# LulinZhang/BRDF-NeRF

Hardware: AMD Instinct MI355X
Metric: train rays/sec (+ MFMA% of roofline), spsbrdf-nerf 64 samples/ray, 1/2/4/8 MI355X (higher is better)
Workload: dtype bf16; 1 GPU; BASELINE config 2: Djibouti-shaped synthetic rays, spsbrdf-nerf lambert train step (pass1 64 + guided 64 samples/ray, F=512, 8 Siren layers, PE10, ds_lambda=10), 4096 rays/GPU/step (4096 rays per global step, weak scaling); rays_per_gpu=4096, n_samples=64, guided_samples=64, parallelism=dp1, settle_steps=224

## Files before the change

### brdf_nerf_amd/csrc/field.h

```cpp
#pragma once
#include "common.h"

#define BN_MAX_PASS 3
#define BN_DPH (3 * BN_MAX_HEADS)
#define BN_SINGLE_HEAD_NTW(NT) ((NT) > 1 ? (NT) / 2 : 1)

struct FieldGeom {
  int F, L, skip, pe_freqs, act;
  int P;
  int KP;
  int NT;
  int BM, waves;
  int dsz;
  int H2;
  int n_heads, n_pass;
  int pass_heads[BN_MAX_PASS];
  int pass_N[BN_MAX_PASS];
  int pass_NTW[BN_MAX_PASS];
  int head_col[BN_MAX_HEADS];
  int C;
  int ch_normal_an, ch_normal_lr;
  int fold;
  int DD, KD, dir_freqs, TD, KT0;
};
// ... 90 lines not shown
  for (int l = 0; l < g.L; ++l) pl->bwd_trunk[l] = l >= 1 ? take(g.F, g.F) : 0;
  pl->bwd_feats = g.fold ? 0 : take(g.F, g.F);
  for (int p = 0; p < g.n_pass; ++p) pl->bwd_head[p] = take(g.F, g.pass_N[p]);
  pl->bwd_pe[0] = take(g.KP, g.F);
  pl->bwd_pe[1] = g.skip > 0 ? take(g.KP, g.F) : 0;
  pl->total = off;
}

struct StashLayout {
  size_t gscale;
  size_t sraw;
  size_t nraw;
  size_t dpre_trunk;
  size_t dpre_head;
  size_t pe;
  size_t dirpe;
  size_t Y[BN_MAX_LAYERS];
  size_t D[BN_MAX_LAYERS];
  size_t feats;
  size_t G[BN_MAX_PASS];
  size_t DG[BN_MAX_PASS];
  size_t dZ[BN_MAX_LAYERS];
  size_t dfeats;
  size_t dG[BN_MAX_PASS];
  size_t gradx;
  size_t sbar;
  size_t sprime;
  size_t gbar_pe;
  size_t adj_delta[BN_MAX_LAYERS];
  size_t adj_a[BN_MAX_LAYERS];
  size_t adj_abar[BN_MAX_LAYERS + 1];
  size_t adj_zbar[BN_MAX_LAYERS];
  size_t wgpart, wgpart_bytes;
  size_t total;
  int64_t Mpad;
};

static inline int64_t bn_wgrad_splits(bool half, int64_t tiles, int64_t Mpad, int64_t *m_per_block) {
  const int64_t stage = half ? 64 : 32;
  const int64_t min_mpb = half ? 512 : 256;
  int64_t n_split = (half ? (Mpad <= 327680 ? BN_W2_BLOCKS : 2 * BN_W2_BLOCKS) : 2048) / (tiles > 0 ? tiles : 1);
  if (n_split < 1) n_split = 1;
  int64_t mpb = ceil_div64(ceil_div64(Mpad, n_split), stage) * stage;
  if (mpb < min_mpb) mpb = min_mpb;
  if (m_per_block) *m_per_block = mpb;
  return ceil_div64(Mpad, mpb);
}
static inline size_t bn_wgpart_bytes(const FieldGeom &g, int64_t Mpad, size_t esz) {
  const bool half = esz != 4;
  const int64_t tl = half ? 256 : 128, ft = (g.F + tl - 1) / tl;
  const int64_t tiles_bound = (2 * g.L + 12) * ft * ft;
  const int64_t grid_bound = half ? 2 * BN_W2_BLOCKS : 2048;
  int64_t slabs = tiles_bound > grid_bound ? tiles_bound : grid_bound;
  const int64_t by_points = tiles_bound * bn_wgrad_splits(half, 1, Mpad, nullptr);
  if (by_points < slabs) slabs = by_points;
  const size_t wg = (size_t)slabs * (size_t)(tl * tl + tl) * 4;
  int64_t sk_splits = ceil_div64(Mpad, g.BM);
  if (sk_splits > 256) sk_splits = 256;
  const size_t sk = (size_t)10 * (size_t)sk_splits * (4 * 512 + 4) * 4;
  return wg > sk ? wg : sk;
}

static inline void bn_make_stash_layout(const FieldGeom &g, int64_t n_points, int BM, size_t esz, StashLayout *s) {
  const size_t dsz = (size_t)g.dsz;
  int64_t Mpad = ceil_div64(n_points, BM) * BM;
  s->Mpad = Mpad;
  size_t off = 0;
  auto take = [&](size_t bytes) { size_t o = off; off += bn_pad(bytes, 256); return o; };
  s->gscale = take(256);
  s->sraw = take((size_t)Mpad * 4);
  s->nraw = take((size_t)Mpad * 16);
  s->dpre_trunk = take((size_t)Mpad * 16);
  s->dpre_head = take((size_t)Mpad * BN_DPH * 4);
  s->pe = take((size_t)Mpad * g.KP * esz);
  s->dirpe = g.KD > 0 ? take((size_t)Mpad * g.KD * esz) : 0;
  for (int l = 0; l < g.L; ++l) s->Y[l] = take((size_t)Mpad * g.F * esz);
  for (int l = 0; l < g.L; ++l) s->D[l] = take((size_t)Mpad * g.F * dsz);
  s->feats = take((size_t)Mpad * g.F * esz);
  for (int p = 0; p < BN_MAX_PASS; ++p) {
    s->G[p] = s->DG[p] = s->dG[p] = 0;
    if (p < g.n_pass) {
      s->G[p] = take((size_t)Mpad * g.F * esz);
      s->DG[p] = take((size_t)Mpad * g.F * dsz);
    }
  }
  for (int l = 0; l < g.L; ++l) s->dZ[l] = take((size_t)Mpad * g.F * esz);
  s->dfeats = take((size_t)Mpad * g.F * esz);
  for (int p = 0; p < g.n_pass; ++p) s->dG[p] = take((size_t)Mpad * g.pass_N[p] * esz);
  s->gradx = s->sbar = s->sprime = s->gbar_pe = 0;
  for (int l = 0; l < BN_MAX_LAYERS; ++l) s->adj_delta[l] = s->adj_a[l] = s->adj_abar[l] = s->adj_zbar[l] = 0;
  s->adj_abar[BN_MAX_LAYERS] = 0;
  if (g.ch_normal_an >= 0) {
    s->gradx = take((size_t)Mpad * 16);
    s->sbar = take((size_t)Mpad * 4);
    s->sprime = take((size_t)Mpad * 4);
    s->gbar_pe = take((size_t)Mpad * g.KP * esz);
    for (int l = 0; l < g.L; ++l) {
      s->adj_delta[l] = take((size_t)Mpad * g.F * esz);
      s->adj_a[l] = take((size_t)Mpad * g.F * esz);
      s->adj_abar[l + 1] = take((size_t)Mpad * g.F * esz);
      s->adj_zbar[l] = take((size_t)Mpad * g.F * esz);
    }
  }
  s->wgpart_bytes = bn_wgpart_bytes(g, Mpad, esz);
  s->wgpart = take(s->wgpart_bytes);
  s->total = off;
}

static inline void bn_stash_layout_at(const FieldGeom &g, const bn_points *pts, int BM, size_t esz, StashLayout *s) {
  const int64_t total = pts->total_points > 0 ? pts->total_points : pts->n_points;
  bn_make_stash_layout(g, total, BM, esz, s);
  const size_t off = (size_t)pts->point_offset;
  if (off == 0) return;
  const size_t dsz = (size_t)g.dsz, F = (size_t)g.F;
  s->sraw += off * 4; s->nraw += off * 16; s->dpre_trunk += off * 16; s->dpre_head += off * BN_DPH * 4;
  s->pe += off * g.KP * esz;
  if (g.KD > 0) s->dirpe += off * g.KD * esz;
  for (int l = 0; l < g.L; ++l) { s->Y[l] += off * F * esz; s->D[l] += off * F * dsz; s->dZ[l] += off * F * esz; }
  s->feats += off * F * esz; s->dfeats += off * F * esz;
  for (int p = 0; p < g.n_pass; ++p) { s->G[p] += off * F * esz; s->DG[p] += off * F * dsz; s->dG[p] += off * g.pass_N[p] * esz; }
  if (g.ch_normal_an >= 0) {
    s->gradx += off * 16; s->sbar += off * 4; s->sprime += off * 4; s->gbar_pe += off * g.KP * esz;
    for (int l = 0; l < g.L; ++l) {
      s->adj_delta[l] += off * F * esz; s->adj_a[l] += off * F * esz; s->adj_abar[l + 1] += off * F * esz; s->adj_zbar[l] += off * F * esz;
    }
  }
  s->Mpad = ceil_div64(pts->n_points, BM) * BM;
}
```

### brdf_nerf_amd/csrc/field_bwd.hip

```cpp
#include "field_kernels.h"
#include "field_wgrad.h"

int bn_field_adjoint_backward(const bn_field_desc *desc, const bn_field_params *params, const void *packed, const bn_points *pts,
                              const float *d_out, void *stash, void *stream);

__device__ unsigned int g_bwd_fault;
unsigned int bn_bwd_fault_read(hipStream_t) {
  unsigned int v = 0u;
  if (hipMemcpyFromSymbol(&v, HIP_SYMBOL(g_bwd_fault), sizeof(unsigned int), 0, hipMemcpyDeviceToHost) != hipSuccess) return 0x80000000u;
  return v;
}
const unsigned int *bn_bwd_fault_ptr() {
  void *p = nullptr;
  return hipGetSymbolAddress(&p, HIP_SYMBOL(g_bwd_fault)) == hipSuccess ? (const unsigned int *)p : nullptr;
}

BN_PH_DEFINE_READER(bn_debug_phase_read_bwd)
BN_CLK_DEFINE(bn_debug_clock_read_bwd)

struct BwdArgs {
  FieldGeom g;
  bn_field_desc d;
  bn_field_params p;
  PackedLayout pl;
// ... 190 lines not shown
  const float gs = chain_scale(A.amax);
  if (tid < 16) WR[tid] = 0;
  if (tid < BM) {
    const int m = tid;
    const int64_t gm = m0 + m;
    float dph[BN_DPH], dpt[4];
    bwd_dpre(A, gm, dph, dpt);
    float *sh = (float *)(A.stash + A.sl.dpre_head) + gm * BN_DPH;
    float *st = (float *)(A.stash + A.sl.dpre_trunk) + gm * 4;
#pragma unroll
    for (int i = 0; i < BN_DPH; ++i) { DPH[m * BN_DPH + i] = dph[i] * gs; sh[i] = dph[i]; }
#pragma unroll
    for (int i = 0; i < 4; ++i) { DPT[m * 4 + i] = dpt[i] * gs; st[i] = dpt[i]; }
  }
  __syncthreads();
  BN_PH(0)

  const int ncol0 = wave * 32 * NT;
  const bool wave_on = ncol0 < F;
  const int n_on = F / (32 * NT) < WAVES ? F / (32 * NT) : WAVES;
  const bool ride = NT == 2 ? true : tile_copy_exact(F, n_on, WAVES);
  f32x16 acc[NT][MT];
  zero_acc<MT, NT>(acc);
  const float zr = (A.an && A.amax) ? gs / grad_scale_from(A.amax + 1, BN_GS_TARGET_ADJ) : 1.f;

  for (int p = 0; p < g.n_pass; ++p) {
    if (g.pass_heads[p] == 2) bwd_head_dG<T, MT, NT, D16>(A, p, ACT, DPH, m0, tile);
    else bwd_head_dG<T, MT, BN_SINGLE_HEAD_NTW(NT), D16>(A, p, ACT, DPH, m0, tile);
    BN_PH(1)
    __syncthreads();
    BN_PH(2)
    BN_PH(3)
    const int KSp = g.pass_N[p] / 16;
    tile_to_global<T>(ACT, LDA, (T *)(A.stash + A.sl.dG[p]) + (size_t)m0 * g.pass_N[p], g.pass_N[p], BM, g.pass_N[p]);
    if (wave_on) gemm_seg<T, MT, NT, DP>(acc, packed + A.pl.bwd_head[p] + (size_t)(ncol0 / 32) * KSp * 512, KSp, ACT, LDA, lane);
    BN_PH(4)
    __syncthreads();
    BN_PH(5)
  }
  if (wave_on && !g.fold) {
#pragma unroll
    for (int nt = 0; nt < NT; ++nt)
#pragma unroll
      for (int gq = 0; gq < 4; ++gq) {
        const int n = ncol0 + nt * 32 + 8 * gq + 4 * h;
#pragma unroll
        for (int mt = 0; mt < MT; ++mt) {
          const int m = mt * 32 + r;
          *(vec4 *)(ACT + (size_t)m * LDA + n) =
              to_vec4(T(), acc[nt][mt][4 * gq], acc[nt][mt][4 * gq + 1], acc[nt][mt][4 * gq + 2], acc[nt][mt][4 * gq + 3]);
        }
      }
  }
  BN_PH(6)
  __syncthreads();
  BN_PH(7)
  BN_PH(8)

  constexpr bool NATZ = Elem<T>::kNativeY;
#ifndef BN_BWD_NO_PINGPONG
  constexpr bool PING = NT == 2 && WAVES == 8 && Elem<T>::kFastMath;
#else
  constexpr bool PING = false;
#endif
  const int grp = wave >> 2;
  const int wave_u = __builtin_amdgcn_readfirstlane(wave);
  DPiece<DK> dpre[NT][MT];
  auto load_D = [&](int lo, int nt0, int nt1) {
    const char *Ds = A.stash + A.sl.D[lo] + (size_t)tile * dtile_bytes<DK>(BM, F);
#pragma unroll
    for (int nt = 0; nt < NT; ++nt)
#pragma unroll
      for (int mt = 0; mt < MT; ++mt) {
        if (nt < nt0 || nt >= nt1) continue;
#ifdef BN_PROBE_NO_D
        if constexpr (std::is_same<DK, DK8>::value) { dpre[nt][mt].w = u32x4{0x80808080u + (unsigned)lane, 0x90909090u, 0xa0a0a0a0u, 0xb0b0b0b0u}; continue; }
#endif
        dpre[nt][mt] = dpiece_load<DK>(Ds + dpiece_off<DK, MT, NT>(wave, nt, mt, lane));
      }
  };
  auto epilogue = [&](int lo, auto top_tag) {
    constexpr bool top = decltype(top_tag)::value;
    const bool nlr = g.ch_normal_lr >= 0;
    const float dscale = (g.act == BN_ACT_SIN && lo == 0) ? 30.f : 1.f;
    const auto Zr = stash_rsrc(A.stash + A.sl.dZ[lo] + (size_t)tile * BM * F * sizeof(T));
    const int voff = lane * 16;
    typedef typename Elem<T>::wide WT;
    constexpr bool ZPRE = sizeof(WT) == 2;
    u32x4 zraw[ZPRE ? NT : 1][ZPRE ? MT : 1][2];
    if constexpr (ZPRE) {
      if (A.an) {
        const WT *Zb = (const WT *)(A.stash + A.sl.adj_zbar[lo]) + (size_t)tile * BM * F;
#pragma unroll
        for (int nt = 0; nt < NT; ++nt)
#pragma unroll
          for (int mt = 0; mt < MT; ++mt)
#pragma unroll
            for (int gp = 0; gp < 2; ++gp) zraw[nt][mt][gp] = stash_load((const u32x4 *)(Zb + native_off8<MT, NT>(wave, nt, mt, gp, lane)));
      }
    }
#pragma unroll
    for (int nt = 0; nt < NT; ++nt)
#pragma unroll
      for (int mt = 0; mt < MT; ++mt) {
        const int m = mt * 32 + r;
#pragma unroll
        for (int gp = 0; gp < 2; ++gp) {
          const int n0 = ncol0 + nt * 32 + 16 * gp + 4 * h;
          float dv[8], v[8];
          dpiece_get<DK>(dpre[nt][mt], gp, g.act, dscale, dv);
#pragma unroll
          for (int e = 0; e < 8; ++e) v[e] = acc[nt][mt][8 * gp + e];
          if constexpr (top) {
            const float ds = DPT[m * 4], a0 = DPT[m * 4 + 1], a1 = DPT[m * 4 + 2], a2 = DPT[m * 4 + 3];
#pragma unroll
            for (int half = 0; half < 2; ++half) {
              const int n = n0 + 8 * half;
              const f32x4 ws = *(const f32x4 *)(A.p.sigma_w + n);
#pragma unroll
              for (int e = 0; e < 4; ++e) v[4 * half + e] += ws[e] * ds;
              if (nlr) {
                const f32x4 wn0 = *(const f32x4 *)(A.p.normal_w + n), wn1 = *(const f32x4 *)(A.p.normal_w + F + n),
                            wn2 = *(const f32x4 *)(A.p.normal_w + 2 * F + n);
#pragma unroll
                for (int e = 0; e < 4; ++e) v[4 * half + e] += wn0[e] * a0 + wn1[e] * a1 + wn2[e] * a2;
              }
            }
          }
#pragma unroll
          for (int e = 0; e < 8; ++e) v[e] *= dv[e];
          if (A.an) {
            float zb[8];
            if constexpr (ZPRE) {
              const auto zq = __builtin_bit_cast(bf16x8, zraw[nt][mt][gp]);
#pragma unroll
              for (int e = 0; e < 8; ++e) zb[e] = (float)zq[e];
            } else {
              ld8((const WT *)(A.stash + A.sl.adj_zbar[lo]) + (size_t)tile * BM * F + native_off8<MT, NT>(wave, nt, mt, gp, lane), zb);
            }
#pragma unroll
            for (int e = 0; e < 8; ++e) v[e] += zb[e] * zr;
          }
          if constexpr (NATZ) {
            const typename Elem<T>::frag q = cvt8(T(), v);
            *(vec4 *)(ACT + (size_t)m * LDA + n0) = __builtin_shufflevector(q, q, 0, 1, 2, 3);
            *(vec4 *)(ACT + (size_t)m * LDA + n0 + 8) = __builtin_shufflevector(q, q, 4, 5, 6, 7);
            stash_store_buf(Zr, voff, ((((wave_u * NT + nt) * MT + mt) * 2 + gp) * 1024), q);
          } else {
            *(vec4 *)(ACT + (size_t)m * LDA + n0) = to_vec4(T(), v[0], v[1], v[2], v[3]);
            *(vec4 *)(ACT + (size_t)m * LDA + n0 + 8) = to_vec4(T(), v[4], v[5], v[6], v[7]);
          }
        }
      }
  };
  {
    if (!g.fold) {
      zero_acc<MT, NT>(acc);
      T *fdst = (T *)(A.stash + A.sl.dfeats) + (size_t)m0 * F;
      if (!ride) tile_to_global<T>(ACT, LDA, fdst, F, BM, F);
      if (wave_on) {
        load_D(g.L - 1, 0, NPRE);
        const size_t off = A.pl.bwd_feats + (size_t)(ncol0 / 32) * KSF * 512;
        if (ride) {
          TileCopyExact<T> zcopy(ACT, LDA, fdst, F, F, tid, WAVES * 64);
          gemm_seg<T, MT, NT, DP>(acc, packed + off, KSF, ACT, LDA, lane, zcopy);
        } else {
          gemm_seg<T, MT, NT, DP>(acc, packed + off, KSF, ACT, LDA, lane);
        }
        load_D(g.L - 1, NPRE, NT);
      }
    } else if (wave_on) {
      load_D(g.L - 1, 0, NT);
    }
    BN_PH(9)
    __syncthreads();
    BN_PH(10)
    if (wave_on) epilogue(g.L - 1, std::true_type());
    BN_PH(11)
    __syncthreads();
    BN_PH(12)
  }
  for (int l = g.L - 1; l >= 1; --l) {
    const int it = g.L - 1 - l;
    const int lo = l - 1;
    zero_acc<MT, NT>(acc);
    T *zdst = (T *)(A.stash + A.sl.dZ[l]) + (size_t)m0 * F;
// ... 100 lines not shown
  bn_make_stash_layout(g, pts->n_points, BM, esz, &a.sl);
  const int64_t tiles = ceil_div64(pts->n_points, BM);
  hipStream_t st = (hipStream_t)stream;
  int rc;
  float *amax = f16m ? (float *)((char *)stash + a.sl.gscale) : nullptr;
  a.amax = amax;
  const unsigned amax_grid = (unsigned)(ceil_div64(pts->n_points, 256) < 1024 ? ceil_div64(pts->n_points, 256) : 1024);
  if (parts & BN_BWD_CHAIN) {
  if (f16m) {
    clear_words_kernel<<<1, 64, 0, st>>>((unsigned int *)amax, 4);
    BN_LAUNCH_CHECK("clear amax");
    if (a.an) {
      grad_amax_kernel<1><<<amax_grid, 256, 0, st>>>(a, amax);
      BN_LAUNCH_CHECK("grad_amax<1>");
    }
  }
  if (a.an) {
    rc = bn_field_adjoint_backward(desc, params, packed, pts, d_out, stash, stream);
    if (rc) return rc;
  }
  if (f16m) {
    grad_amax_kernel<0><<<amax_grid, 256, 0, st>>>(a, amax);
    BN_LAUNCH_CHECK("grad_amax<0>");
  }
  rc = [&]() -> int { BN_DISPATCH_TILE(desc->dtype, g, launch_bwd, (a, tiles, st)); }();
  if (rc) return rc;
  }

  const StashLayout &sl = a.sl;
  char *S = (char *)stash;
  const int F = g.F, P0 = g.P;
  WgradArgs w;
  w.n_jobs = 0; w.Mpad = sl.Mpad; w.tile0[0] = 0; w.amax = amax; w.part = nullptr; w.n_split = 1;
  int scale_sel = 1;
  int b_native = 0;
  int a_native = 0;
  int part = BN_BWD_WGRAD_TRUNK;
  auto add = [&](const void *A_, int lda, int a0, const void *B_, int ldb, int b0, float *C, int ldc, float *bias, int N, int K) {
    if (!C || !(parts & part)) return;
    WgradJob &j = w.job[w.n_jobs];
    j.scale_sel = scale_sel;
    j.b_native = (b_native ? WG_B_NATIVE : 0) | (a_native ? WG_A_NATIVE : 0); j.b_bm = BM; j.b_F = F; j.b_bm_shift = BM == 128 ? 7 : 6;
    j.A = A_; j.B = B_; j.C = C; j.bias = bias; j.lda = lda; j.ldb = ldb; j.ldc = ldc; j.a_col0 = a0; j.b_col0 = b0; j.N = N; j.K = K;
    w.tile0[w.n_jobs + 1] = w.tile0[w.n_jobs] + ((N + 127) / 128) * ((K + 127) / 128);
    ++w.n_jobs;
  };
  const int naty = bf ? 1 : 0;
  a_native = naty;
  for (int l = 0; l < g.L; ++l) {
    const void *dZ = S + sl.dZ[l];
    b_native = 0;
    if (l == 0) add(dZ, F, 0, S + sl.pe, g.KP, 0, G->trunk_w[l], P0, G->trunk_b[l], F, P0);
    else if (l == g.skip) {
      add(dZ, F, 0, S + sl.pe, g.KP, 0, G->trunk_w[l], F + P0, G->trunk_b[l], F, P0);
      b_native = naty;
      add(dZ, F, 0, S + sl.Y[l - 1], F, 0, G->trunk_w[l] ? G->trunk_w[l] + P0 : nullptr, F + P0, nullptr, F, F);
    } else {
      b_native = naty;
      add(dZ, F, 0, S + sl.Y[l - 1], F, 0, G->trunk_w[l], F, G->trunk_b[l], F, F);
    }
  }
  a_native = 0;
  b_native = naty;
  part = BN_BWD_WGRAD_HEADS;
  if (!g.fold) add(S + sl.dfeats, F, 0, S + sl.Y[g.L - 1], F, 0, G->feats_w, F, G->feats_b, F, F);
  part = BN_BWD_WGRAD_TRUNK;
  b_native = 0;
  if (a.an) {
    scale_sel = 2;
    for (int l = 0; l < g.L; ++l) {
      const void *dl = S + sl.adj_delta[l];
      if (l == 0) add(dl, F, 0, S + sl.gbar_pe, g.KP, 0, G->trunk_w[l], P0, nullptr, F, P0);
      else if (l == g.skip) {
        add(dl, F, 0, S + sl.gbar_pe, g.KP, 0, G->trunk_w[l], F + P0, nullptr, F, P0);
        add(dl, F, 0, S + sl.adj_abar[l], F, 0, G->trunk_w[l] ? G->trunk_w[l] + P0 : nullptr, F + P0, nullptr, F, F);
      } else add(dl, F, 0, S + sl.adj_abar[l], F, 0, G->trunk_w[l], F, nullptr, F, F);
    }
  }
  scale_sel = 1;
  part = BN_BWD_WGRAD_HEADS;
  for (int hd = 0; hd < g.n_heads; ++hd) {
    const int p = hd / 2, hl = hd % 2;
    b_native = g.fold ? naty : 0;
    add(S + sl.dG[p], g.pass_N[p], hl * g.H2, S + (g.fold ? sl.Y[g.L - 1] : sl.feats), F, 0, G->head_w1[hd], F, G->head_b1[hd], g.H2, F);
  }
  if (g.DD > 0 && G->head0_wdir) {
    b_native = 0; scale_sel = 1;
    add(S + sl.dG[0], g.pass_N[0], 0, S + sl.dirpe, g.KD, 0, G->head0_wdir, (int)G->head0_wdir_ld, nullptr, g.H2, g.DD);
  }
  if (g.TD > 0 && G->head1_wt) {
    b_native = 0; scale_sel = 1;
    add(S + sl.dG[0], g.pass_N[0], g.H2, S + sl.dirpe, g.KD, g.KT0, G->head1_wt, (int)G->head1_wt_ld, nullptr, g.H2, g.TD);
  }
  BN_REQUIRE(w.n_jobs <= BN_MAX_WGRAD_JOBS, "field_backward: too many wgrad jobs");
  float *wgpart = (float *)(S + sl.wgpart);
  if (w.n_jobs > 0)
    if (int e = bn_launch_wgrad(w, bf, f16m, sl.Mpad, wgpart, sl.wgpart_bytes, st)) return e;
  if (!(parts & BN_BWD_SKINNY)) return 0;
  SkinnyArgs s;
  s.n_jobs = 0; s.Mpad = sl.Mpad; s.amax = amax; s.part = nullptr;
  for (int i = 0; i < BN_MAX_SKINNY_JOBS; ++i) { s.job[i].scale_sel = 0; s.job[i].unit_dpre = 0; }
  {
    SkinnyJob &j = s.job[s.n_jobs];
    j.X = S + sl.Y[g.L - 1]; j.ldx = F; j.x_col0 = 0; j.K = F; j.dpre = (const float *)(S + sl.dpre_trunk); j.ldp = 4; j.p_col0 = 0;
    j.nc = g.ch_normal_lr >= 0 ? 4 : 1; j.native = 0;
    if (naty) { j.native = 1; j.bm = BM; j.ntw = g.NT; j.tstride = BM * F; }
    for (int c = 0; c < 4; ++c) { j.out[c] = nullptr; j.bias[c] = nullptr; }
    j.out[0] = G->sigma_w; j.bias[0] = G->sigma_b;
    if (g.ch_normal_lr >= 0) {
      BN_REQUIRE(G->normal_w && G->normal_b, "field_backward: normal grads missing");
      for (int c = 0; c < 3; ++c) { j.out[1 + c] = G->normal_w + (size_t)c * F; j.bias[1 + c] = G->normal_b + c; }
    }
    if (j.out[0]) ++s.n_jobs;
  }
  if (a.an && G->sigma_w) {
    SkinnyJob &j = s.job[s.n_jobs++];
// ... 40 lines not shown
```

### brdf_nerf_amd/csrc/field_kernels.h

```cpp
#pragma once
#include "field.h"
#include "instrument.h"

typedef __attribute__((ext_vector_type(4))) unsigned int u32x4;
typedef __attribute__((ext_vector_type(2))) unsigned int u32x2;
template <typename V> __device__ __forceinline__ void stash_store(V *p, const V &v) {
#ifdef BN_NO_NT_STASH
  *p = v;
#else
  __builtin_nontemporal_store(v, p);
#endif
}
template <typename V> __device__ __forceinline__ V stash_load(const V *p) {
#ifdef BN_NO_NT_STASH
  return *p;
#else
  return __builtin_nontemporal_load(p);
#endif
}

__device__ __forceinline__ auto stash_rsrc(const void *base) {
  const unsigned long long b = (unsigned long long)base;
  const unsigned int lo = __builtin_amdgcn_readfirstlane((unsigned int)b), hi = __builtin_amdgcn_readfirstlane((unsigned int)(b >> 32));
  return __builtin_amdgcn_make_buffer_rsrc((void *)(((unsigned long long)hi << 32) | lo), 0, 0x7fffffff, 0x00020000);
// ... 246 lines not shown
    if constexpr (std::is_same<std::decay_t<Side>, NoSide>::value) {
      if (KS == 16) { gemm_fixed<T, MT, NTW, D, 16, 0>(acc, wp, KS, 0, bsrc, ldb, lane, NoMid()); return; }
    }
  }
  gemm_seg<T, MT, NTW, DP>(acc, wp, KS, bsrc, ldb, lane, side);
}

template <int MT, int NTW> __device__ __forceinline__ void zero_acc(f32x16 (&acc)[NTW][MT]) {
#pragma unroll
  for (int nt = 0; nt < NTW; ++nt)
#pragma unroll
    for (int mt = 0; mt < MT; ++mt)
#pragma unroll
      for (int i = 0; i < 16; ++i) acc[nt][mt][i] = 0.f;
}

template <int MT, int NTW> __device__ __forceinline__ size_t native_off8(int wave, int nt, int mt, int gp, int lane) {
  return ((((size_t)(wave * NTW + nt) * MT + mt) * 2 + gp) * 64 + lane) * 8;
}
__device__ __forceinline__ bf16x8 cvt8(bf16, const float (&v)[8]) {
  bf16x8 o;
#pragma unroll
  for (int i = 0; i < 8; ++i) o[i] = (bf16)v[i];
  return o;
}
__device__ __forceinline__ f16x8 cvt8(f16, const float (&v)[8]) {
  const f32x8 f = {v[0], v[1], v[2], v[3], v[4], v[5], v[6], v[7]};
  return __builtin_convertvector(f, f16x8);
}
__device__ __forceinline__ f32x8 cvt8(float, const float (&v)[8]) {
  const f32x8 f = {v[0], v[1], v[2], v[3], v[4], v[5], v[6], v[7]};
  return f;
}
__device__ __forceinline__ void st_frag(bf16 *p, const bf16x8 &o) { stash_store((bf16x8 *)p, o); }
__device__ __forceinline__ void st_frag(f16 *p, const f16x8 &o) { stash_store((f16x8 *)p, o); }
__device__ __forceinline__ void st_frag(float *p, const f32x8 &o) {
  stash_store((f32x4 *)p, f32x4{o[0], o[1], o[2], o[3]});
  stash_store((f32x4 *)(p + 4), f32x4{o[4], o[5], o[6], o[7]});
}
template <typename T> __device__ __forceinline__ void st8(T *p, const float (&v)[8]) { st_frag(p, cvt8(T(), v)); }
__device__ __forceinline__ void ld8(const bf16 *p, float (&v)[8]) {
  const bf16x8 o = stash_load((const bf16x8 *)p);
#pragma unroll
  for (int i = 0; i < 8; ++i) v[i] = (float)o[i];
}
__device__ __forceinline__ void ld8(const f16 *p, float (&v)[8]) {
  const f16x8 o = stash_load((const f16x8 *)p);
#pragma unroll
  for (int i = 0; i < 8; ++i) v[i] = (float)o[i];
}
__device__ __forceinline__ void ld8(const float *p, float (&v)[8]) {
  const f32x4 a = stash_load((const f32x4 *)p), b = stash_load((const f32x4 *)(p + 4));
#pragma unroll
  for (int i = 0; i < 4; ++i) { v[i] = a[i]; v[4 + i] = b[i]; }
}

template <typename DK> struct DPiece { u32x4 w; };
template <> struct DPiece<DK16> { u32x4 w[2]; };
template <> struct DPiece<DK32> { f32x4 v[4]; };
template <typename DK> __host__ __device__ constexpr size_t dk_bytes() { return std::is_same<DK, DK32>::value ? 4 : (std::is_same<DK, DK16>::value ? 2 : 1); }
template <typename DK> __host__ __device__ constexpr size_t dtile_bytes(int BM, int F) { return (size_t)BM * F * dk_bytes<DK>(); }
template <typename DK, int MT, int NTW> __device__ __forceinline__ size_t dpiece_off(int wave, int nt, int mt, int lane) {
  return ((size_t)(wave * NTW + nt) * MT + mt) * (1024 * dk_bytes<DK>()) + (size_t)lane * (std::is_same<DK, DK32>::value ? 64 : 16);
}
__device__ __forceinline__ unsigned int d8_pack4(float c0, float c1, float c2, float c3) {
  const unsigned int lo = __builtin_bit_cast(unsigned int, __builtin_amdgcn_cvt_pknorm_i16(c0, c1)),
// ... 102 lines not shown
```

### brdf_nerf_amd/csrc/field_wgrad.h

```cpp
#pragma once
#include <hip/hip_runtime.h>
#include <stdint.h>

struct WgradJob {
  const void *A;
  const void *B;
  float *C;
  float *bias;
  int lda, ldb, ldc;
  int a_col0, b_col0;
  int N, K;
  int scale_sel;
  int b_native;
  int b_bm, b_F;
  int b_bm_shift;
};
#define WG_B_NATIVE 1
#define WG_A_NATIVE 2
#define BN_MAX_WGRAD_JOBS 44
struct WgradArgs {
  WgradJob job[BN_MAX_WGRAD_JOBS];
  int tile0[BN_MAX_WGRAD_JOBS + 1];
  int n_jobs;
  int64_t Mpad;
  int m_per_block;
  const float *amax;
  float *part;
  int n_split;
  int chain_next[BN_MAX_WGRAD_JOBS];
  unsigned char head[BN_MAX_WGRAD_JOBS];
};
#define WG_SLAB256 (256 * 256 + 256)
#define WG_SLAB128 (128 * 128 + 128)
#define SK_SLAB (4 * 512 + 4)

struct SkinnyJob {
  const void *X;
  const float *dpre;
  int ldx, x_col0, K, ldp, p_col0, nc;
  int native;
  int bm, ntw, tstride;
  float *out[4];
  float *bias[4];
  int scale_sel;
  int unit_dpre;
};
#define BN_MAX_SKINNY_JOBS 10
struct SkinnyArgs {
  SkinnyJob job[BN_MAX_SKINNY_JOBS];
  int n_jobs;
  int64_t Mpad;
  int m_per_block;
  const float *amax;
  float *part;
};

int bn_launch_wgrad(WgradArgs &wv, bool bf, bool f16m, int64_t Mpad, float *part, size_t part_bytes, hipStream_t st);
int bn_launch_skinny(SkinnyArgs &sv, bool bf, bool f16m, int64_t Mpad, int64_t m_per_block, float *part, size_t part_bytes, hipStream_t st);
unsigned int bn_bwd_fault_read(hipStream_t st);
```

### brdf_nerf_amd/csrc/field_wgrad.hip

```cpp
#include "field_kernels.h"
#include "field_wgrad.h"


__device__ __forceinline__ float wg_unscale(const float *amax, int sel) {
  if (amax == nullptr || sel == 0) return 1.f;
  return 1.f / (sel == 1 ? chain_scale(amax) : grad_scale_from(amax + 1, BN_GS_TARGET_ADJ));
}

#define WG_BK 32
template <typename T> struct WgTile;
template <> struct WgTile<float> { static constexpr int LD = 128 + 4; };

template <typename T> __device__ __forceinline__ typename Elem<T>::frag wg_frag(const T *tile, int mm, int col0, int lane);
template <> __device__ __forceinline__ f32x8 wg_frag<float>(const float *tile, int mm, int col0, int lane) {
  constexpr int LD = WgTile<float>::LD;
  const int h = lane >> 5, r = lane & 31;
  f32x8 f;
#pragma unroll
  for (int j = 0; j < 8; ++j) f[j] = tile[(size_t)(mm + 2 * j + h) * LD + col0 + r];
  return f;
}

template <typename T> __global__ __launch_bounds__(256) void wgrad_kernel(const WgradArgs A) {
  constexpr int LD = WgTile<T>::LD;
// ... 60 lines not shown
    if (do_bias) {
#pragma unroll 8
      for (int row = 0; row < WG_BK; ++row) bsum += (float)sA[row * LD + tid];
    }
  }
  float *P = A.part + ((size_t)blockIdx.x * gridDim.y + blockIdx.y) * WG_SLAB128;
#pragma unroll
  for (int a = 0; a < 2; ++a)
#pragma unroll
    for (int b = 0; b < 2; ++b)
#pragma unroll
      for (int q = 0; q < 4; ++q)
        *(f32x4 *)(P + (size_t)(((((wave * 2 + a) * 2 + b) * 4 + q) * 64 + lane) * 4)) =
            f32x4{acc[a][b][4 * q], acc[a][b][4 * q + 1], acc[a][b][4 * q + 2], acc[a][b][4 * q + 3]};
  if (do_bias) P[128 * 128 + tid] = bsum;
}

__device__ __attribute__((aligned(16))) unsigned short w2_zeros[8];
#define W2_LD (256 + 32)
#define W2_BK 64
#define W2_STAGE (W2_BK * W2_LD)
__device__ __forceinline__ int w2_swz(int row) { return ((row >> 1) & 3) << 1; }
template <typename T> __device__ __forceinline__ typename Elem<T>::frag w2_frag(const T *tile, int mm, int col0, int lane) {
  const int h = lane >> 5, grp = (lane >> 4) & 1, i = lane & 15, q = i >> 2, p = i & 3;
  const int s_lo = (4 * grp + p) ^ w2_swz(8 * h + q);
  const int d_hi = 4 * W2_LD + ((((s_lo ^ 4) - s_lo)) << 2);
  const T *a = tile + (size_t)(mm + 8 * h + q) * W2_LD + (((col0 >> 2) + s_lo) << 2);
  typedef __attribute__((address_space(3))) s16x4 lds_v4;
  const s16x4 lo = __builtin_amdgcn_ds_read_tr16_b64_v4i16((lds_v4 *)a);
  const s16x4 hi = __builtin_amdgcn_ds_read_tr16_b64_v4i16((lds_v4 *)(a + d_hi));
  union { s16x4 s[2]; typename Elem<T>::frag b; } u;
  u.s[0] = lo; u.s[1] = hi;
  return u.b;
}

__device__ __forceinline__ float frag_sum8(float s, const bf16x8 &f) {
  typedef __attribute__((ext_vector_type(2))) __bf16 bf16x2;
  const bf16x2 one = {(__bf16)1.f, (__bf16)1.f};
  s = __builtin_amdgcn_fdot2_f32_bf16(__builtin_shufflevector(f, f, 0, 1), one, s, false);
  s = __builtin_amdgcn_fdot2_f32_bf16(__builtin_shufflevector(f, f, 2, 3), one, s, false);
  s = __builtin_amdgcn_fdot2_f32_bf16(__builtin_shufflevector(f, f, 4, 5), one, s, false);
  s = __builtin_amdgcn_fdot2_f32_bf16(__builtin_shufflevector(f, f, 6, 7), one, s, false);
  return s;
}
__device__ __forceinline__ float frag_sum8(float s, const f16x8 &f) {
  typedef __attribute__((ext_vector_type(2))) _Float16 f16x2;
  const f16x2 one = {(_Float16)1.f, (_Float16)1.f};
  s = __builtin_amdgcn_fdot2(__builtin_shufflevector(f, f, 0, 1), one, s, false);
  s = __builtin_amdgcn_fdot2(__builtin_shufflevector(f, f, 2, 3), one, s, false);
  s = __builtin_amdgcn_fdot2(__builtin_shufflevector(f, f, 4, 5), one, s, false);
  s = __builtin_amdgcn_fdot2(__builtin_shufflevector(f, f, 6, 7), one, s, false);
  return s;
}
__device__ __forceinline__ float frag_sum8(float s, const f32x8 &f) {
#pragma unroll
  for (int j = 0; j < 8; ++j) s += f[j];
  return s;
}

#if defined(BN_PHASE_TIMING) && defined(BN_PHASE_TIMING_WGRAD)
BN_PH_DEFINE_READER(bn_debug_phase_read_wgrad)
#define WG_PH_DECL BN_PH_DECL
#define WG_PH(i) BN_PH(i)
#define WG_PH_FLUSH BN_PH_FLUSH
#else
#define WG_PH_DECL
#define WG_PH(i)
#define WG_PH_FLUSH
#endif
#ifndef W2_WAVES
#define W2_WAVES 8
#endif
#define W2_RA (256 / ((W2_WAVES / 2) * 32))
template <typename T, int NBV, bool BNAT, bool ANAT>
__device__ __forceinline__ void w2_body(const WgradJob &J, int n0, int k0, int64_t mb, int64_t me, T *sA, T *sB, float *P) {
  typedef typename Elem<T>::frag frag_t;
  const int tid = threadIdx.x, lane = tid & 63, wave = tid >> 6, wr = wave >> 1, wc = wave & 1;
  const T *gA = (const T *)J.A + J.a_col0 + n0;
  const T *gB = (const T *)J.B + J.b_col0 + k0;
  constexpr int RPP = W2_WAVES * 2;
  constexpr int NC = W2_BK / RPP;
  const int row0 = tid >> 5, cc = (tid & 31) * 8;
  const bool a_ok = n0 + cc < J.N, b_ok = k0 + cc < J.K;
  const int scol = (((cc >> 2) ^ w2_swz(row0)) << 2);
  const int nr = lane & 31, nh = lane >> 5, nswz = w2_swz(nr);
  static_assert(W2_BK / (W2_WAVES * 2) == 4, "native staging: 4 wave-instructions per wave and stage");
  const int mtn = (BNAT || ANAT) ? J.b_bm / 32 : 1, ncb = (BNAT || ANAT) ? J.b_F / 32 : 1;
  int cbg = (k0 >> 5) + wave;
  cbg = cbg < ncb ? cbg : ncb - 1;
  const int boff0 = (cbg * mtn * 2 * 64 + lane) * 8;
// ... 20 lines not shown
    for (int c = 0; c < NC; ++c) gload1(m, c);
  };
  auto sstore1 = [&](int buf, int c) {
    if (ANAT) {
      T *rowp = sA + buf * W2_STAGE + (32 * (c & 1) + nr) * W2_LD;
      const int sl0 = lslot0 + 4 * ((c >> 1) & 1);
      const auto s02 = __builtin_amdgcn_permlane32_swap(ra[c][0], ra[c][2], false, false);
      const auto s13 = __builtin_amdgcn_permlane32_swap(ra[c][1], ra[c][3], false, false);
      *(u32x4 *)(rowp + ((sl0 ^ nswz) << 2)) = u32x4{s02[0], s13[0], s02[1], s13[1]};
    } else {
      *(u32x4 *)(sA + buf * W2_STAGE + (row0 + RPP * c) * W2_LD + scol) = ra[c];
    }
    if (BNAT) {
      T *rowp = sB + buf * W2_STAGE + (32 * (c & 1) + nr) * W2_LD;
      const int sl0 = lslot0 + 4 * ((c >> 1) & 1);
      const auto s02 = __builtin_amdgcn_permlane32_swap(rb[c][0], rb[c][2], false, false);
      const auto s13 = __builtin_amdgcn_permlane32_swap(rb[c][1], rb[c][3], false, false);
      *(u32x4 *)(rowp + ((sl0 ^ nswz) << 2)) = u32x4{s02[0], s13[0], s02[1], s13[1]};
    } else {
      *(u32x4 *)(sB + buf * W2_STAGE + (row0 + RPP * c) * W2_LD + scol) = rb[c];
    }
  };
  auto sstore = [&](int buf) {
#pragma unroll
    for (int c = 0; c < NC; ++c) sstore1(buf, c);
  };
  f32x16 acc[W2_RA][4];
#pragma unroll
  for (int a = 0; a < W2_RA; ++a)
#pragma unroll
    for (int b = 0; b < 4; ++b)
#pragma unroll
      for (int i = 0; i < 16; ++i) acc[a][b][i] = 0.f;
  constexpr int BA = W2_RA / 2;
  const bool do_bias = J.bias != nullptr && k0 == 0;
  float bsum[BA];
#pragma unroll
  for (int a = 0; a < BA; ++a) bsum[a] = 0.f;
  WG_PH_DECL
  auto compute = [&](int buf, int64_t m_next2) {
    const T *cA = sA + buf * W2_STAGE, *cB = sB + buf * W2_STAGE;
    frag_t fa[2][W2_RA], fb[2][NBV > 0 ? NBV : 1];
    auto frags = [&](int set, int mm) {
#pragma unroll
      for (int a = 0; a < W2_RA; ++a) fa[set][a] = w2_frag<T>(cA, mm, wr * (W2_RA * 32) + a * 32, lane);
#pragma unroll
      for (int b = 0; b < NBV; ++b) fb[set][b] = w2_frag<T>(cB, mm, wc * 128 + b * 32, lane);
    };
    frags(0, 0);
#pragma unroll
    for (int i = 0; i < W2_BK / 16; ++i) {
      const int cur = i & 1;
      if (i + 1 < W2_BK / 16) frags(cur ^ 1, (i + 1) * 16);
      __builtin_amdgcn_sched_barrier(0);
#pragma unroll
      for (int a = 0; a < W2_RA; ++a)
#pragma unroll
        for (int b = 0; b < NBV; ++b) mma32(acc[a][b], fa[cur][a], fb[cur][b]);
      {
#pragma unroll
        for (int a = 0; a < BA; ++a) {
          const u32x4 f0 = __builtin_bit_cast(u32x4, fa[cur][a]), f1 = __builtin_bit_cast(u32x4, fa[cur][BA + a]);
          bsum[a] = frag_sum8(bsum[a], __builtin_bit_cast(frag_t, wc ? f1 : f0));
        }
      }
      {
        constexpr int CPS = NC / (W2_BK / 16) > 0 ? NC / (W2_BK / 16) : 1;
#pragma unroll
        for (int q = 0; q < CPS; ++q) {
          const int c = i * CPS + q;
          if (c < NC) { sstore1(buf ^ 1, c); gload1(m_next2, c); }
        }
      }
      __builtin_amdgcn_sched_barrier(0);
    }
  };
  gload(mb);
  sstore(0);
#pragma unroll
  for (int c = 0; c < NC; ++c) {
    __builtin_amdgcn_sched_barrier(0);
    gload1(mb + W2_BK, c);
  }
  __builtin_amdgcn_sched_barrier(0);
  WG_PH(14)
  int buf = 0;
  for (int64_t m = mb; m < me; m += W2_BK) {
    __syncthreads();
    WG_PH(3)
    compute(buf, m + 2 * W2_BK);
    WG_PH(0)
    buf ^= 1;
  }
  const int r = lane & 31, h = lane >> 5;
#pragma unroll
  for (int a = 0; a < W2_RA; ++a)
#pragma unroll
    for (int b = 0; b < 4; ++b)
#pragma unroll
      for (int q = 0; q < 4; ++q)
        *(f32x4 *)(P + (size_t)(((((wave * W2_RA + a) * 4 + b) * 4 + q) * 64 + lane) * 4)) =
            f32x4{acc[a][b][4 * q], acc[a][b][4 * q + 1], acc[a][b][4 * q + 2], acc[a][b][4 * q + 3]};
  if (do_bias) {
#pragma unroll
    for (int a = 0; a < BA; ++a) {
      const float v = bsum[a] + __shfl_xor(bsum[a], 32);
      if (h == 0) P[256 * 256 + wr * (W2_RA * 32) + (wc * BA + a) * 32 + r] = v;
    }
  }
  WG_PH(4)
  WG_PH_FLUSH
}

template <typename T>
__global__ __launch_bounds__(W2_WAVES * 64, W2_WAVES == 8 ? 2 : 1) void wgrad256_kernel(const WgradArgs A, int n_split, int n_blocks) {
  extern __shared__ __attribute__((aligned(16))) char smem_w[];
  T *sA = (T *)smem_w;
  T *sB = sA + 2 * W2_STAGE;
  const int per = n_blocks / 8;
  const int lid = (int)((blockIdx.x % 8) * per + blockIdx.x / 8);
  const int total_tiles = A.tile0[A.n_jobs];
  if (lid >= total_tiles * n_split) return;
  const int split = lid / total_tiles, tt = lid % total_tiles;
  int jb = 0;
  while (jb + 1 < A.n_jobs && tt >= A.tile0[jb + 1]) ++jb;
  const WgradJob &J = A.job[jb];
  const int t = tt - A.tile0[jb];
  const int tiles_k = (J.K + 255) / 256;
  const int n0 = (t / tiles_k) * 256, k0 = (t % tiles_k) * 256;
  const int64_t mb = (int64_t)split * A.m_per_block;
  const int64_t me = mb + A.m_per_block < A.Mpad ? mb + A.m_per_block : A.Mpad;
  if (mb >= me) return;
  const int wc = (threadIdx.x >> 6) & 1;
  const int cols = J.K - k0 - wc * 128;
  float *P = A.part + ((size_t)tt * n_split + split) * WG_SLAB256;
#ifdef BN_CLOCK_STAMP_WGRAD
  BN_CLK_BEGIN
#endif
  if (J.b_native & WG_A_NATIVE) {
    if (J.b_native & WG_B_NATIVE) {
      if (cols >= 65) w2_body<T, 4, true, true>(J, n0, k0, mb, me, sA, sB, P);
      else if (cols >= 33) w2_body<T, 2, true, true>(J, n0, k0, mb, me, sA, sB, P);
// ... 108 lines not shown
#pragma unroll
      for (int c = 0; c < 4; ++c) {
        const float d = J.unit_dpre ? 1.f : dp[c];
#pragma unroll
        for (int e = 0; e < 8; ++e) s[c][e] += d * x[e];
        bs[c] += d;
      }
    }
  }
  for (int turn = 0; turn < nrg; ++turn) {
    if (rg == turn) {
#pragma unroll
      for (int c = 0; c < 4; ++c)
        if (c < J.nc) {
#pragma unroll
          for (int e = 0; e < 8; ++e) red[c * 512 + cg * 8 + e] += s[c][e];
          if (cg == 0) red[4 * 512 + c] += bs[c];
        }
    }
    __syncthreads();
  }
  }
  __syncthreads();
  float *SP = A.part + ((size_t)blockIdx.y * gridDim.x + blockIdx.x) * SK_SLAB;
  for (int i = tid; i < J.nc * J.K; i += 256) {
    const int c = i / J.K, k = i % J.K;
    SP[c * 512 + k] = red[c * 512 + k];
  }
  if (tid < 4) SP[4 * 512 + tid] = tid < J.nc ? red[4 * 512 + tid] : 0.f;
}

template <int TILE> __global__ __launch_bounds__(256) void wgrad_reduce_kernel(const WgradArgs A) {
  constexpr int NB = TILE / 64;
  constexpr int SLAB = TILE * TILE + TILE;
  constexpr int SUBS = TILE * TILE / 4 / 256;
  const int tt = blockIdx.x / SUBS, sub = blockIdx.x % SUBS, tid = threadIdx.x;
  int jb = 0;
  while (jb + 1 < A.n_jobs && tt >= A.tile0[jb + 1]) ++jb;
  if (!A.head[jb]) return;
  const WgradJob &J = A.job[jb];
  const int t = tt - A.tile0[jb];
  const int tiles_k = (J.K + TILE - 1) / TILE;
  const int n0 = (t / tiles_k) * TILE, k0 = (t % tiles_k) * TILE;
  const int ns = A.n_split;
  {
    const int idx4 = sub * 256 + tid;
    const int lane = idx4 & 63, q = (idx4 >> 6) & 3, b = (idx4 >> 8) % NB, a = ((idx4 >> 8) / NB) & 1, wave = (idx4 >> 8) / (NB * 2);
    f32x4 v = {0.f, 0.f, 0.f, 0.f};
    for (int jj = jb; jj >= 0; jj = A.chain_next[jj]) {
      const float osc = wg_unscale(A.amax, A.job[jj].scale_sel);
      const float *P = A.part + (size_t)(A.tile0[jj] + t) * ns * SLAB + (size_t)idx4 * 4;
      f32x4 sum = {0.f, 0.f, 0.f, 0.f};
      int sp = 0;
      for (; sp + 8 <= ns; sp += 8) {
        f32x4 x[8];
#pragma unroll
        for (int u = 0; u < 8; ++u) x[u] = *(const f32x4 *)(P + (size_t)(sp + u) * SLAB);
#pragma unroll
        for (int u = 0; u < 8; ++u) sum += x[u];
      }
      for (; sp < ns; ++sp) sum += *(const f32x4 *)(P + (size_t)sp * SLAB);
      v += sum * osc;
    }
    const int r = lane & 31, h = lane >> 5, wr = wave >> 1, wc = wave & 1;
    const int k = k0 + wc * (TILE / 2) + b * 32 + r, nb = n0 + wr * 64 + a * 32 + 8 * q + 4 * h;
#pragma unroll
    for (int e = 0; e < 4; ++e)
      if (nb + e < J.N && k < J.K) J.C[(size_t)(nb + e) * J.ldc + k] += v[e];
  }
  if (sub == 0 && k0 == 0 && tid < TILE && n0 + tid < J.N) {
    float v = 0.f;
    float *dst = nullptr;
    for (int jj = jb; jj >= 0; jj = A.chain_next[jj]) {
      if (!A.job[jj].bias) continue;
      dst = A.job[jj].bias;
      const float osc = wg_unscale(A.amax, A.job[jj].scale_sel);
      const float *P = A.part + (size_t)(A.tile0[jj] + t) * ns * SLAB + TILE * TILE + tid;
      float sum = 0.f;
      for (int sp = 0; sp < ns; ++sp) sum += P[(size_t)sp * SLAB];
      v += sum * osc;
    }
    if (dst) dst[n0 + tid] += v;
  }
}

__global__ __launch_bounds__(256) void skinny_reduce_kernel(const SkinnyArgs A, int n_split) {
  __shared__ float part[8][32], bpart[256];
  const int jb = blockIdx.x, c = blockIdx.y, k0 = blockIdx.z * 32, tid = threadIdx.x, kk = tid & 31, g = tid >> 5;
  const SkinnyJob &J = A.job[jb];
  if (c >= J.nc || !J.out[c] || k0 >= J.K) return;
  for (int j2 = 0; j2 < jb; ++j2)
    for (int c2 = 0; c2 < A.job[j2].nc; ++c2)
      if (A.job[j2].out[c2] == J.out[c]) return;
  float v = 0.f, vb = 0.f;
  for (int j2 = jb; j2 < A.n_jobs; ++j2)
    for (int c2 = 0; c2 < A.job[j2].nc; ++c2) {
      if (A.job[j2].out[c2] != J.out[c]) continue;
      const float osc = wg_unscale(A.amax, A.job[j2].scale_sel);
      const float *P = A.part + (size_t)j2 * n_split * SK_SLAB;
      const bool col = k0 + kk < A.job[j2].K;
      float sum = 0.f;
      int sp = g;
      for (; sp + 56 < n_split; sp += 64) {
// ... 119 lines not shown
```

Baseline: 620,300 rays/s.

## Compute bias-gradient column sums in backward kernel instead of wgrad GEMM

Moves bias-gradient accumulation out of the half-precision 256-tile weight-gradient kernel. The backward field kernel now writes per-tile column sums of dZ/dfeats/dG into a new stash buffer, using DPP cross-lane reductions. The wgrad reduce kernel sums those partials across tiles. This removes the per-MFMA-step fdot2 bias work from the wgrad inner loop and shrinks the partial slabs. In exchange it adds reductions and extra global stores to the backward epilogue and a new stash allocation.

```diff
diff --git a/brdf_nerf_amd/csrc/field.h b/brdf_nerf_amd/csrc/field.h
--- a/brdf_nerf_amd/csrc/field.h
+++ b/brdf_nerf_amd/csrc/field.h
@@ -146,6 +146,8 @@
   size_t adj_abar[BN_MAX_LAYERS + 1];
   size_t adj_zbar[BN_MAX_LAYERS];
   size_t wgpart, wgpart_bytes;
+  size_t bpart;
+  int bpart_rows;
   size_t total;
   int64_t Mpad;
 };
@@ -168,7 +170,7 @@
   int64_t slabs = tiles_bound > grid_bound ? tiles_bound : grid_bound;
   const int64_t by_points = tiles_bound * bn_wgrad_splits(half, 1, Mpad, nullptr);
   if (by_points < slabs) slabs = by_points;
-  const size_t wg = (size_t)slabs * (size_t)(tl * tl + tl) * 4;
+  const size_t wg = (size_t)slabs * (size_t)(half ? tl * tl : tl * tl + tl) * 4;
   int64_t sk_splits = ceil_div64(Mpad, g.BM);
   if (sk_splits > 256) sk_splits = 256;
   const size_t sk = (size_t)10 * (size_t)sk_splits * (4 * 512 + 4) * 4;
@@ -218,6 +220,8 @@
   }
   s->wgpart_bytes = bn_wgpart_bytes(g, Mpad, esz);
   s->wgpart = take(s->wgpart_bytes);
+  s->bpart_rows = g.L + 1 + g.n_pass;
+  s->bpart = esz != 4 ? take((size_t)(Mpad / BM) * s->bpart_rows * g.F * 4) : 0;
   s->total = off;
 }
 
diff --git a/brdf_nerf_amd/csrc/field_bwd.hip b/brdf_nerf_amd/csrc/field_bwd.hip
--- a/brdf_nerf_amd/csrc/field_bwd.hip
+++ b/brdf_nerf_amd/csrc/field_bwd.hip
@@ -246,6 +246,15 @@
     BN_PH(2)
     BN_PH(3)
     const int KSp = g.pass_N[p] / 16;
+    if constexpr (Elem<T>::kNativeY) {
+      float *bp = (float *)(A.stash + A.sl.bpart) + ((size_t)tile * A.sl.bpart_rows + g.L + 1 + p) * F;
+      for (int c = tid; c < g.pass_N[p]; c += WAVES * 64) {
+        float s = 0.f;
+#pragma unroll 8
+        for (int m = 0; m < BM; ++m) s += (float)ACT[(size_t)m * LDA + c];
+        bp[c] = s;
+      }
+    }
     tile_to_global<T>(ACT, LDA, (T *)(A.stash + A.sl.dG[p]) + (size_t)m0 * g.pass_N[p], g.pass_N[p], BM, g.pass_N[p]);
     if (wave_on) gemm_seg<T, MT, NT, DP>(acc, packed + A.pl.bwd_head[p] + (size_t)(ncol0 / 32) * KSp * 512, KSp, ACT, LDA, lane);
     BN_PH(4)
@@ -258,12 +267,16 @@
 #pragma unroll
       for (int gq = 0; gq < 4; ++gq) {
         const int n = ncol0 + nt * 32 + 8 * gq + 4 * h;
+        float bs[4];
 #pragma unroll
         for (int mt = 0; mt < MT; ++mt) {
           const int m = mt * 32 + r;
-          *(vec4 *)(ACT + (size_t)m * LDA + n) =
-              to_vec4(T(), acc[nt][mt][4 * gq], acc[nt][mt][4 * gq + 1], acc[nt][mt][4 * gq + 2], acc[nt][mt][4 * gq + 3]);
+          const vec4 q = to_vec4(T(), acc[nt][mt][4 * gq], acc[nt][mt][4 * gq + 1], acc[nt][mt][4 * gq + 2], acc[nt][mt][4 * gq + 3]);
+          *(vec4 *)(ACT + (size_t)m * LDA + n) = q;
+          if constexpr (Elem<T>::kNativeY) colsum_add(bs, q, mt == 0);
         }
+        if constexpr (Elem<T>::kNativeY)
+          colsum_store(bs, (float *)(A.stash + A.sl.bpart) + ((size_t)tile * A.sl.bpart_rows + g.L) * F + n, lane);
       }
   }
   BN_PH(6)
@@ -314,13 +327,14 @@
       }
     }
 #pragma unroll
-    for (int nt = 0; nt < NT; ++nt)
-#pragma unroll
-      for (int mt = 0; mt < MT; ++mt) {
-        const int m = mt * 32 + r;
-#pragma unroll
-        for (int gp = 0; gp < 2; ++gp) {
-          const int n0 = ncol0 + nt * 32 + 16 * gp + 4 * h;
+    for (int nt = 0; nt < NT; ++nt) {
+#pragma unroll
+      for (int gp = 0; gp < 2; ++gp) {
+        const int n0 = ncol0 + nt * 32 + 16 * gp + 4 * h;
+        float bs[8];
+#pragma unroll
+        for (int mt = 0; mt < MT; ++mt) {
+          const int m = mt * 32 + r;
           float dv[8], v[8];
           dpiece_get<DK>(dpre[nt][mt], gp, g.act, dscale, dv);
 #pragma unroll
@@ -360,12 +374,15 @@
             *(vec4 *)(ACT + (size_t)m * LDA + n0) = __builtin_shufflevector(q, q, 0, 1, 2, 3);
             *(vec4 *)(ACT + (size_t)m * LDA + n0 + 8) = __builtin_shufflevector(q, q, 4, 5, 6, 7);
             stash_store_buf(Zr, voff, ((((wave_u * NT + nt) * MT + mt) * 2 + gp) * 1024), q);
+            colsum_add(bs, q, mt == 0);
           } else {
             *(vec4 *)(ACT + (size_t)m * LDA + n0) = to_vec4(T(), v[0], v[1], v[2], v[3]);
             *(vec4 *)(ACT + (size_t)m * LDA + n0 + 8) = to_vec4(T(), v[4], v[5], v[6], v[7]);
           }
         }
-      }
+        if constexpr (NATZ) colsum_store(bs, (float *)(A.stash + A.sl.bpart) + ((size_t)tile * A.sl.bpart_rows + lo) * F + n0, lane);
+      }
+    }
   };
   {
     if (!g.fold) {
@@ -532,16 +549,18 @@
   const int F = g.F, P0 = g.P;
   WgradArgs w;
   w.n_jobs = 0; w.Mpad = sl.Mpad; w.tile0[0] = 0; w.amax = amax; w.part = nullptr; w.n_split = 1;
+  w.bpart = (const float *)(S + sl.bpart); w.bp_tiles = (int)(sl.Mpad / BM); w.bp_rows = sl.bpart_rows; w.bp_F = F;
   int scale_sel = 1;
   int b_native = 0;
   int a_native = 0;
   int part = BN_BWD_WGRAD_TRUNK;
+  int bias_row = -1;
   auto add = [&](const void *A_, int lda, int a0, const void *B_, int ldb, int b0, float *C, int ldc, float *bias, int N, int K) {
     if (!C || !(parts & part)) return;
     WgradJob &j = w.job[w.n_jobs];
     j.scale_sel = scale_sel;
     j.b_native = (b_native ? WG_B_NATIVE : 0) | (a_native ? WG_A_NATIVE : 0); j.b_bm = BM; j.b_F = F; j.b_bm_shift = BM == 128 ? 7 : 6;
-    j.A = A_; j.B = B_; j.C = C; j.bias = bias; j.lda = lda; j.ldb = ldb; j.ldc = ldc; j.a_col0 = a0; j.b_col0 = b0; j.N = N; j.K = K;
+    j.A = A_; j.B = B_; j.C = C; j.bias = bias; j.bias_row = bias_row; j.lda = lda; j.ldb = ldb; j.ldc = ldc; j.a_col0 = a0; j.b_col0 = b0; j.N = N; j.K = K;
     w.tile0[w.n_jobs + 1] = w.tile0[w.n_jobs] + ((N + 127) / 128) * ((K + 127) / 128);
     ++w.n_jobs;
   };
@@ -550,6 +569,7 @@
   for (int l = 0; l < g.L; ++l) {
     const void *dZ = S + sl.dZ[l];
     b_native = 0;
+    bias_row = l;
     if (l == 0) add(dZ, F, 0, S + sl.pe, g.KP, 0, G->trunk_w[l], P0, G->trunk_b[l], F, P0);
     else if (l == g.skip) {
       add(dZ, F, 0, S + sl.pe, g.KP, 0, G->trunk_w[l], F + P0, G->trunk_b[l], F, P0);
@@ -563,6 +583,7 @@
   a_native = 0;
   b_native = naty;
   part = BN_BWD_WGRAD_HEADS;
+  bias_row = g.L;
   if (!g.fold) add(S + sl.dfeats, F, 0, S + sl.Y[g.L - 1], F, 0, G->feats_w, F, G->feats_b, F, F);
   part = BN_BWD_WGRAD_TRUNK;
   b_native = 0;
@@ -582,6 +603,7 @@
   for (int hd = 0; hd < g.n_heads; ++hd) {
     const int p = hd / 2, hl = hd % 2;
     b_native = g.fold ? naty : 0;
+    bias_row = g.L + 1 + p;
     add(S + sl.dG[p], g.pass_N[p], hl * g.H2, S + (g.fold ? sl.Y[g.L - 1] : sl.feats), F, 0, G->head_w1[hd], F, G->head_b1[hd], g.H2, F);
   }
   if (g.DD > 0 && G->head0_wdir) {
diff --git a/brdf_nerf_amd/csrc/field_kernels.h b/brdf_nerf_amd/csrc/field_kernels.h
--- a/brdf_nerf_amd/csrc/field_kernels.h
+++ b/brdf_nerf_amd/csrc/field_kernels.h
@@ -302,6 +302,29 @@
   const f32x8 f = {v[0], v[1], v[2], v[3], v[4], v[5], v[6], v[7]};
   return f;
 }
+template <int CTRL, int ROWS> __device__ __forceinline__ float dpp_take(float v) {
+  return __builtin_bit_cast(float, __builtin_amdgcn_update_dpp(0, __builtin_bit_cast(int, v), CTRL, ROWS, 0xf, false));
+}
+__device__ __forceinline__ float rsum32(float v) {
+  v += dpp_take<0xB1, 0xf>(v);
+  v += dpp_take<0x4E, 0xf>(v);
+  v += dpp_take<0x141, 0xf>(v);
+  v += dpp_take<0x140, 0xf>(v);
+  v += dpp_take<0x142, 0xa>(v);
+  return v;
+}
+template <int NV, typename V> __device__ __forceinline__ void colsum_add(float (&s)[NV], const V &q, bool first, int e0 = 0) {
+#pragma unroll
+  for (int e = 0; e < (int)(sizeof(V) / sizeof(q[0])); ++e) s[e0 + e] = first ? (float)q[e] : s[e0 + e] + (float)q[e];
+}
+template <int NV> __device__ __forceinline__ void colsum_store(float (&s)[NV], float *dst, int lane) {
+#pragma unroll
+  for (int e = 0; e < NV; ++e) s[e] = rsum32(s[e]);
+  if ((lane & 31) == 31) {
+    *(f32x4 *)dst = f32x4{s[0], s[1], s[2], s[3]};
+    if constexpr (NV == 8) *(f32x4 *)(dst + 8) = f32x4{s[4], s[5], s[6], s[7]};
+  }
+}
 __device__ __forceinline__ void st_frag(bf16 *p, const bf16x8 &o) { stash_store((bf16x8 *)p, o); }
 __device__ __forceinline__ void st_frag(f16 *p, const f16x8 &o) { stash_store((f16x8 *)p, o); }
 __device__ __forceinline__ void st_frag(float *p, const f32x8 &o) {
diff --git a/brdf_nerf_amd/csrc/field_wgrad.h b/brdf_nerf_amd/csrc/field_wgrad.h
--- a/brdf_nerf_amd/csrc/field_wgrad.h
+++ b/brdf_nerf_amd/csrc/field_wgrad.h
@@ -7,6 +7,7 @@
   const void *B;
   float *C;
   float *bias;
+  int bias_row;
   int lda, ldb, ldc;
   int a_col0, b_col0;
   int N, K;
@@ -29,8 +30,10 @@
   int n_split;
   int chain_next[BN_MAX_WGRAD_JOBS];
   unsigned char head[BN_MAX_WGRAD_JOBS];
+  const float *bpart;
+  int bp_tiles, bp_rows, bp_F;
 };
-#define WG_SLAB256 (256 * 256 + 256)
+#define WG_SLAB256 (256 * 256)
 #define WG_SLAB128 (128 * 128 + 128)
 #define SK_SLAB (4 * 512 + 4)
 
diff --git a/brdf_nerf_amd/csrc/field_wgrad.hip b/brdf_nerf_amd/csrc/field_wgrad.hip
--- a/brdf_nerf_amd/csrc/field_wgrad.hip
+++ b/brdf_nerf_amd/csrc/field_wgrad.hip
@@ -116,30 +116,6 @@
   union { s16x4 s[2]; typename Elem<T>::frag b; } u;
   u.s[0] = lo; u.s[1] = hi;
   return u.b;
-}
-
-__device__ __forceinline__ float frag_sum8(float s, const bf16x8 &f) {
-  typedef __attribute__((ext_vector_type(2))) __bf16 bf16x2;
-  const bf16x2 one = {(__bf16)1.f, (__bf16)1.f};
-  s = __builtin_amdgcn_fdot2_f32_bf16(__builtin_shufflevector(f, f, 0, 1), one, s, false);
-  s = __builtin_amdgcn_fdot2_f32_bf16(__builtin_shufflevector(f, f, 2, 3), one, s, false);
-  s = __builtin_amdgcn_fdot2_f32_bf16(__builtin_shufflevector(f, f, 4, 5), one, s, false);
-  s = __builtin_amdgcn_fdot2_f32_bf16(__builtin_shufflevector(f, f, 6, 7), one, s, false);
-  return s;
-}
-__device__ __forceinline__ float frag_sum8(float s, const f16x8 &f) {
-  typedef __attribute__((ext_vector_type(2))) _Float16 f16x2;
-  const f16x2 one = {(_Float16)1.f, (_Float16)1.f};
-  s = __builtin_amdgcn_fdot2(__builtin_shufflevector(f, f, 0, 1), one, s, false);
-  s = __builtin_amdgcn_fdot2(__builtin_shufflevector(f, f, 2, 3), one, s, false);
-  s = __builtin_amdgcn_fdot2(__builtin_shufflevector(f, f, 4, 5), one, s, false);
-  s = __builtin_amdgcn_fdot2(__builtin_shufflevector(f, f, 6, 7), one, s, false);
-  return s;
-}
-__device__ __forceinline__ float frag_sum8(float s, const f32x8 &f) {
-#pragma unroll
-  for (int j = 0; j < 8; ++j) s += f[j];
-  return s;
 }
 
 #if defined(BN_PHASE_TIMING) && defined(BN_PHASE_TIMING_WGRAD)
@@ -226,11 +202,6 @@
     for (int b = 0; b < 4; ++b)
 #pragma unroll
       for (int i = 0; i < 16; ++i) acc[a][b][i] = 0.f;
-  constexpr int BA = W2_RA / 2;
-  const bool do_bias = J.bias != nullptr && k0 == 0;
-  float bsum[BA];
-#pragma unroll
-  for (int a = 0; a < BA; ++a) bsum[a] = 0.f;
   WG_PH_DECL
   auto compute = [&](int buf, int64_t m_next2) {
     const T *cA = sA + buf * W2_STAGE, *cB = sB + buf * W2_STAGE;
@@ -251,13 +222,6 @@
       for (int a = 0; a < W2_RA; ++a)
 #pragma unroll
         for (int b = 0; b < NBV; ++b) mma32(acc[a][b], fa[cur][a], fb[cur][b]);
-      {
-#pragma unroll
-        for (int a = 0; a < BA; ++a) {
-          const u32x4 f0 = __builtin_bit_cast(u32x4, fa[cur][a]), f1 = __builtin_bit_cast(u32x4, fa[cur][BA + a]);
-          bsum[a] = frag_sum8(bsum[a], __builtin_bit_cast(frag_t, wc ? f1 : f0));
-        }
-      }
       {
         constexpr int CPS = NC / (W2_BK / 16) > 0 ? NC / (W2_BK / 16) : 1;
 #pragma unroll
@@ -286,7 +250,6 @@
     WG_PH(0)
     buf ^= 1;
   }
-  const int r = lane & 31, h = lane >> 5;
 #pragma unroll
   for (int a = 0; a < W2_RA; ++a)
 #pragma unroll
@@ -295,13 +258,6 @@
       for (int q = 0; q < 4; ++q)
         *(f32x4 *)(P + (size_t)(((((wave * W2_RA + a) * 4 + b) * 4 + q) * 64 + lane) * 4)) =
             f32x4{acc[a][b][4 * q], acc[a][b][4 * q + 1], acc[a][b][4 * q + 2], acc[a][b][4 * q + 3]};
-  if (do_bias) {
-#pragma unroll
-    for (int a = 0; a < BA; ++a) {
-      const float v = bsum[a] + __shfl_xor(bsum[a], 32);
-      if (h == 0) P[256 * 256 + wr * (W2_RA * 32) + (wc * BA + a) * 32 + r] = v;
-    }
-  }
   WG_PH(4)
   WG_PH_FLUSH
 }
@@ -476,7 +432,7 @@
 
 template <int TILE> __global__ __launch_bounds__(256) void wgrad_reduce_kernel(const WgradArgs A) {
   constexpr int NB = TILE / 64;
-  constexpr int SLAB = TILE * TILE + TILE;
+  constexpr int SLAB = TILE == 256 ? WG_SLAB256 : WG_SLAB128;
   constexpr int SUBS = TILE * TILE / 4 / 256;
   const int tt = blockIdx.x / SUBS, sub = blockIdx.x % SUBS, tid = threadIdx.x;
   int jb = 0;
@@ -512,7 +468,41 @@
     for (int e = 0; e < 4; ++e)
       if (nb + e < J.N && k < J.K) J.C[(size_t)(nb + e) * J.ldc + k] += v[e];
   }
-  if (sub == 0 && k0 == 0 && tid < TILE && n0 + tid < J.N) {
+  if constexpr (TILE == 256) {
+    if (k0 != 0 || sub >= 16) return;
+    __shared__ float bred[16][16];
+    const int kk = tid & 15, g = tid >> 4, n = n0 + sub * 16 + kk;
+    const size_t ts = (size_t)A.bp_rows * A.bp_F;
+    float v = 0.f;
+    float *dst = nullptr;
+    for (int jj = jb; jj >= 0; jj = A.chain_next[jj]) {
+      const WgradJob &Q = A.job[jj];
+      if (!Q.bias) continue;
+      dst = Q.bias;
+      const float osc = wg_unscale(A.amax, Q.scale_sel);
+      const float *B = A.bpart + (size_t)Q.bias_row * A.bp_F + Q.a_col0 + (n < Q.N ? n : 0);
+      float sum = 0.f;
+      int pt = g;
+      for (; pt + 240 < A.bp_tiles; pt += 256) {
+        float x[16];
+#pragma unroll
+        for (int u = 0; u < 16; ++u) x[u] = B[(size_t)(pt + 16 * u) * ts];
+#pragma unroll
+        for (int u = 0; u < 16; ++u) sum += x[u];
+      }
+      for (; pt < A.bp_tiles; pt += 16) sum += B[(size_t)pt * ts];
+      __syncthreads();
+      bred[g][kk] = sum;
+      __syncthreads();
+      if (g == 0) {
+        float t2 = 0.f;
+#pragma unroll
+        for (int q = 0; q < 16; ++q) t2 += bred[q][kk];
+        v += t2 * osc;
+      }
+    }
+    if (g == 0 && dst && n < J.N) dst[n] += v;
+  } else if (sub == 0 && k0 == 0 && tid < TILE && n0 + tid < J.N) {
     float v = 0.f;
     float *dst = nullptr;
     for (int jj = jb; jj >= 0; jj = A.chain_next[jj]) {
```

Measured after the change: 605,300 rays/s. 0.976x the previous value.
